# mryndzionek/composable-sdr

Measured on AMD Instinct MI355X. Metric: MS/s CF32 throughput, 256-ch PFB+FM pipeline, higher is better.
Workload: dtype f32; 1 GPU; cfg3: 256-ch firpfbch(m=7,As=80)+dcBlocker+freqdem(kf=0.3) on synthetic CF32, AGC off (-a 0), 262144 frames/step (512 MiB in, 256 MiB out), HBM-resident; channels=256, demod=fm, mix=False, route=fused-256|k_tile256<FM>, preheat_steps=10762, collective=none, rccl_ranks=1

## Files before the change

### composable_sdr_amd/csrc/capi.hip

```cpp
#include "../../include/csdr.h"
#include "csdr_internal.h"
#include "fused.h"

#include <cmath>
#include <cstdio>
#include <cstring>
#include <new>

namespace csdr {
const char *last_error();
}
using namespace csdr;

namespace {

struct DevGuard {
    int prev = -1; bool ok = true;
    DevGuard() = default;
    explicit DevGuard(int dev) { select(dev); }
    void select(int dev) {
        if (hipGetDevice(&prev) != hipSuccess) { ok = false; return; }
        if (dev >= 0 && dev != prev && hipSetDevice(dev) != hipSuccess) ok = false;
    }
    ~DevGuard() { if (prev >= 0) (void)hipSetDevice(prev); }
// ... 983 lines not shown
        h->d_theta = nco_freq_word(pfb_premix_freq(M));
        h->tab_len = nco_period(h->d_theta, 1u << 17);
        if ((r = chain_alloc(h, &h->d_taps, h->taps.size()))) return fail(r);
        CSDR_HIP_CLEAN(hipMemcpy(h->d_taps, h->taps.data(), sizeof(float) * h->taps.size(), hipMemcpyHostToDevice), csdr_chain_destroy(h));
        if (h->tab_len) {
            std::vector<float2> tab(h->tab_len);
            for (uint32_t i = 0; i < h->tab_len; i++) { float c, s; nco_phasor(i * h->d_theta, &c, &s); tab[i] = make_float2(c, s); }
            if ((r = chain_alloc(h, &h->d_nco_tab, h->tab_len))) return fail(r);
            CSDR_HIP_CLEAN(hipMemcpy(h->d_nco_tab, tab.data(), sizeof(float2) * h->tab_len, hipMemcpyHostToDevice), csdr_chain_destroy(h));
        }
        std::vector<float2> tw(M);
        for (uint32_t i = 0; i < M; i++) {
            double a = -2.0 * 3.14159265358979323846 * (double)i / (double)M;
            tw[i] = make_float2((float)std::cos(a), (float)std::sin(a));
        }
        if ((r = chain_alloc(h, &h->d_tw, M))) return fail(r);
        CSDR_HIP_CLEAN(hipMemcpy(h->d_tw, tw.data(), sizeof(float2) * M, hipMemcpyHostToDevice), csdr_chain_destroy(h));
    }
    if (cfg->agc_threshold_db != 0.0f && (r = chain_alloc(h, &h->d_agc, C))) return fail(r);
    if (cfg->demod == CSDR_DEMOD_FM && ((r = chain_alloc(h, &h->d_rp[0], C)) || (r = chain_alloc(h, &h->d_rp[1], C)))) return fail(r);

    const DcParams *dcp = cfg->dc_block ? &h->dc : nullptr;
    const RouteRow *route = route_select(M, h->p, G, cfg->flags, dcp);
    if (route->M == 4096 && (C != M || (cfg->mix && cfg->demod == CSDR_DEMOD_NONE && cfg->agc_threshold_db == 0.0f && !am)))
        route = route_select(M, h->p, G, cfg->flags | CSDR_FLAG_FORCE_GENERIC, dcp);
    if (route->create) {
        const bool agc_on = cfg->agc_threshold_db != 0.0f;
        FusedConfig fc{};
        fc.M = M; fc.p = h->p; fc.C = C; fc.c0 = c0; fc.max_nf = h->max_nf; fc.G = G;
        fc.dc_block = cfg->dc_block != 0; fc.dc = h->dc;
        fc.fm = cfg->demod == CSDR_DEMOD_FM && !agc_on; fc.fm_ref = h->fm_ref;
        fc.mix = cfg->mix != 0 && !agc_on; fc.taps = h->taps.data(); fc.d_theta = h->d_theta; fc.cus = h->n_cus;
        if ((r = route->create(fc, &h->plan))) return fail(r);
        h->path = std::string(route->path_prefix) + h->plan->name() + (G > 1 ? "+interleaved-shard" : "") + (agc_on ? "+agc" : "");
        h->timed_kernel = h->plan->name();
        if (agc_on) {
            const bool tm_possible = !(cfg->flags & CSDR_FLAG_AGC_SEQUENTIAL) && h->max_nf >= 4096u &&
                                     (C % 64u == 0 || (C < 64u && 64u % C == 0));
            h->a_guard = tm_possible ? agc_tail_tm_guard(C) : 0;
            if ((r = chain_alloc(h, &h->d_A, (size_t)C * h->max_nf + 2 * h->a_guard))) return fail(r);
            if (h->a_guard) {
                CSDR_HIP_CLEAN(hipMemset(h->d_A, 0, sizeof(float2) * h->a_guard), csdr_chain_destroy(h));
                CSDR_HIP_CLEAN(hipMemset(h->d_A + h->a_guard + (size_t)C * h->max_nf, 0, sizeof(float2) * h->a_guard), csdr_chain_destroy(h));
            }
            if (cfg->mix && (r = chain_alloc(h, &h->d_B, (size_t)C * h->max_nf))) return fail(r);
        }
    } else {
        h->path = "generic";
        const bool use1024 = G == 1 && pfb1024_supported(M, h->p) && !(cfg->mix && cfg->agc_threshold_db == 0.0f) && !diag_env("CSDR_NO_PFB1024");
        h->timed_kernel = M > 1 ? (use1024 ? "k_pfb1024" : "k_pfb_fir") : "k_dc_apply";
        if (use1024) h->path = "generic+pfb1024";
        if (M > 1) {
            if ((r = chain_alloc(h, &h->d_u, (size_t)(h->p - 1) * M + h->max_nx)) || (r = chain_alloc(h, &h->d_hist_tmp, (size_t)(h->p - 1) * M))) return fail(r);
        }
        if ((r = chain_alloc(h, &h->d_A, h->max_nx)) || (r = chain_alloc(h, &h->d_B, use1024 && h->max_nx < 2048 ? 2048 : h->max_nx))) return fail(r);
        if (M > 1 && cfg->dc_block && (r = dctile_create(h->dc, h->max_nx, &h->dctile))) return fail(r);
        h->mix_identity = M > 1 && G == 1 && C == M && cfg->mix && cfg->demod == CSDR_DEMOD_NONE && cfg->agc_threshold_db == 0.0f &&
                          h->dctile && !(cfg->flags & CSDR_FLAG_NO_MIX_IDENTITY) && !am;
        if (h->mix_identity) {
            if ((r = chain_alloc(h, &h->d_u0, (size_t)(h->p - 1) + h->max_nf)) || (r = chain_alloc(h, &h->d_u0hist, 2 * (h->p - 1)))) return fail(r);
            h->path = "generic+mix-identity"; h->timed_kernel = (M % 4096u == 0) ? "k_dc_fold" : "k_dc_tile";
        }
        h->mix_identity_shard = M > 1 && (G == 2 || G == 4 || G == 8) && (uint64_t)C * G == M && cfg->mix && cfg->demod == CSDR_DEMOD_NONE && cfg->agc_threshold_db == 0.0f &&
                                h->dctile && !(cfg->flags & CSDR_FLAG_NO_MIX_IDENTITY) && !am && M % 4096u == 0 && (M / G) % 512u == 0 &&
                                h->p <= 33u && h->dc.beta > 0.f;
        if (h->mix_identity_shard) {
            if ((r = chain_alloc(h, &h->d_u0hist, 2 * (size_t)(h->p - 1) * G))) return fail(r);
// ... 616 lines not shown
```

### composable_sdr_amd/csrc/fused.h

```cpp
#pragma once
#include "csdr_internal.h"

namespace csdr {

struct FusedConfig {
    uint32_t M, p, C, c0, max_nf;
    uint32_t G = 1;
    bool dc_block; DcParams dc;
    bool fm; float fm_ref;
    bool mix;
    const float *taps;
    uint32_t d_theta;
    uint32_t cus = 256;
};

struct FusedCall {
    const float2 *d_in;
    void *d_out;
    uint32_t nf;
    uint32_t theta0;
    bool indep = false;
    hipEvent_t ev_tail = nullptr;
    bool tile_major = false;
};

struct ChainPlan {
    FusedConfig cfg;
    uint32_t cus;
    uint64_t frames_done = 0;
    int cur = 0;
    void *d_premix = nullptr;
    DeviceBuffers mem;

    explicit ChainPlan(const FusedConfig &c) : cfg(c), cus(c.cus) {}
    virtual ~ChainPlan() = default;

    int process(const FusedCall &call, hipStream_t s, KernelTimer *timer);
    int reset(hipStream_t s) { cur = 0; frames_done = 0; return reset_state(s); }
    void seek(uint64_t frames) { frames_done = frames; }
    virtual const char *name() const = 0;
    virtual bool tile_major_ok(uint32_t nf) const = 0;

    virtual void keep_tail() {}
    virtual bool can_overlap(uint32_t nf) const { (void)nf; return false; }
    virtual bool tail_recorded() const { return false; }
    virtual int status(unsigned *st) { *st = 0; return 0; }
    virtual int trace(unsigned long long *out, uint32_t ntiles) { (void)out; (void)ntiles; return 0; }

protected:
    std::vector<float2> premix_table() const;
    virtual int reset_state(hipStream_t s) = 0;
    virtual int run(const FusedCall &call, void *out, hipStream_t s, KernelTimer *timer) = 0;
};

template <class Plan> int make_plan(const FusedConfig &cfg, ChainPlan **out)
{
    Plan *p = new Plan(cfg);
    if (int r = p->init()) { delete p; return r; }
    *out = p;
    return 0;
}

bool plan256_supported(uint32_t M, uint32_t p);
int  plan256_create(const FusedConfig &cfg, ChainPlan **out);
bool plan64_supported(uint32_t M, uint32_t p);
int  plan64_create(const FusedConfig &cfg, ChainPlan **out);
bool plan1024_supported(uint32_t M, uint32_t p);
int  plan1024_create(const FusedConfig &cfg, ChainPlan **out);
bool plan4096_supported(uint32_t M, uint32_t p);
int  plan4096_create(const FusedConfig &cfg, ChainPlan **out);

int  run256_v2_launch(const void *run_args, bool fm, unsigned G, unsigned nruns, hipStream_t s);
int  run256_v2_blocks_per_cu(bool fm);
// ... 60 lines not shown
```

### composable_sdr_amd/csrc/fused_common.h

```cpp
#pragma once
#include "fused.h"

#include <cmath>
#include <cstdlib>
#include <vector>

namespace csdr {
namespace {

constexpr int M256 = 256;
constexpr int P = 14;
constexpr int NB = 16;
constexpr int FS_X = 272;
constexpr int FS_Z = 289;
constexpr int RS_Z = 18;
constexpr int RS_Y = 17;
constexpr int LDS_F2 = 16 * FS_Z;
constexpr int E_OFF = 4096;
constexpr int LOOKBACK = 10;
constexpr unsigned SPIN_LIMIT = 1u << 24;

typedef unsigned long long u64;
typedef float v2f __attribute__((ext_vector_type(2)));

// ... 320 lines not shown
    return f ? r : make_float2(0.f, 0.f);
}


constexpr int WU = 6;

struct RunSplit {
    uint32_t rps, nslots;
    uint32_t base[8], tiles[8];
};
__host__ __device__ __forceinline__ void run_range(const RunSplit &sp, uint32_t w, uint32_t &first, uint32_t &last)
{
    const uint32_t s = w / sp.rps, i = w - s * sp.rps;
    first = sp.base[s] + (uint32_t)((unsigned long long)i * sp.tiles[s] / sp.rps);
    last = sp.base[s] + (uint32_t)((unsigned long long)(i + 1) * sp.tiles[s] / sp.rps);
}

struct RunArgs {
    TileArgs t;
    RunSplit split;
    PhaseK pk;
    uint32_t nruns;
    float l2beta;
    uint32_t prio_div;
    uint32_t trace_light;
    const float4 *prev_tail;
    uint32_t indep;
    uint32_t pair_align;
    uint32_t wu_batch6;
    uint32_t wu, wu_rot;
    uint32_t tile_step;
    uint32_t nowu;
    float2 *cpre, *side;
};
constexpr int DCFIX_F = 113;

__device__ __forceinline__ float2 wg_sum(float2 v, float2 *red, int tid)
{
#pragma unroll
    for (int d = 32; d >= 1; d >>= 1) { v.x += __shfl_xor(v.x, d); v.y += __shfl_xor(v.y, d); }
    if ((tid & 63) == 0) red[tid >> 6] = v;
    __syncthreads();
    const float2 r = cadd(cadd(red[0], red[1]), cadd(red[2], red[3]));
    __syncthreads();
    return r;
}

__device__ __forceinline__ void row_scan4(float &x0, float &x1, float &x2, float &x3, float &s0, float &s1, float &s2, float &s3,
                                          float b1, float b2, float b4, float b8, float na)
{
    asm volatile(
        "v_mov_b32_e32 %4, %0\n\t"
        "v_mov_b32_e32 %5, %1\n\t"
        "v_mov_b32_e32 %6, %2\n\t"
        "v_mov_b32_e32 %7, %3\n\t"
        "v_fmac_f32_dpp %4, %4, %8 row_shr:1 row_mask:0xf bank_mask:0xf\n\t"
        "v_fmac_f32_dpp %5, %5, %8 row_shr:1 row_mask:0xf bank_mask:0xf\n\t"
        "v_fmac_f32_dpp %6, %6, %8 row_shr:1 row_mask:0xf bank_mask:0xf\n\t"
        "v_fmac_f32_dpp %7, %7, %8 row_shr:1 row_mask:0xf bank_mask:0xf\n\t"
        "v_fmac_f32_dpp %4, %4, %9 row_shr:2 row_mask:0xf bank_mask:0xf\n\t"
        "v_fmac_f32_dpp %5, %5, %9 row_shr:2 row_mask:0xf bank_mask:0xf\n\t"
        "v_fmac_f32_dpp %6, %6, %9 row_shr:2 row_mask:0xf bank_mask:0xf\n\t"
        "v_fmac_f32_dpp %7, %7, %9 row_shr:2 row_mask:0xf bank_mask:0xf\n\t"
        "v_fmac_f32_dpp %4, %4, %10 row_shr:4 row_mask:0xf bank_mask:0xf\n\t"
        "v_fmac_f32_dpp %5, %5, %10 row_shr:4 row_mask:0xf bank_mask:0xf\n\t"
        "v_fmac_f32_dpp %6, %6, %10 row_shr:4 row_mask:0xf bank_mask:0xf\n\t"
// ... 64 lines not shown
```

### composable_sdr_amd/csrc/kernels_fused.hip

```cpp
#include "fused_common.h"
#include <cstring>

namespace csdr {

namespace {

#define STAMP(i) do { if (A.trace && tid == 0) A.trace[(size_t)b * 16 + (i)] = __builtin_amdgcn_s_memtime(); } while (0)

template <bool FM>
__global__ __launch_bounds__(256) void k_tile256(TileArgs A)
{
    __shared__ __attribute__((aligned(16))) float2 R[LDS_F2];
    __shared__ float2 tw_s[M256];
    __shared__ float2 Tt[2][16];
    __shared__ float2 carry_s[2];
    __shared__ unsigned tile_s;

    const int tid = threadIdx.x;
    if (tid == 0) tile_s = atomicAdd(A.ticket, 1u);
    tw_s[tid] = A.tw[tid];
    __syncthreads();
    const unsigned b = tile_s;
    if (b >= A.nb) return;
    STAMP(0);
// ... 256 lines not shown
            if (end < base || sp.tiles[k] < 8 * cus) ok = false;
            base = end;
        }
        if (ok) return sp;
    }
    sp = RunSplit{};
    sp.rps = nruns; sp.nslots = 1; sp.base[0] = 0; sp.tiles[0] = nb;
    return sp;
}

__global__ __launch_bounds__(256) void k_save_tail(const float4 *__restrict__ src, float4 *__restrict__ dst)
{
    const unsigned i = blockIdx.x * 256u + threadIdx.x;
    dst[i] = src[i];
}

__global__ __launch_bounds__(64) void k_shard_gather(const float *__restrict__ src, float *__restrict__ dst, uint32_t c0, uint32_t G, uint32_t rem,
                                                     uint32_t nf, uint32_t t0, uint32_t w)
{
    const uint32_t m = blockIdx.x;
    for (uint32_t i = threadIdx.x; i < rem * w; i += 64) dst[((size_t)m * nf + t0) * w + i] = src[(size_t)(c0 + G * m) * rem * w + i];
}

struct FusedPlan : ChainPlan {
    using ChainPlan::ChainPlan;
    std::string kernel;
    uint32_t max_nb = 0, epoch = 0;
    float *d_taps = nullptr;
    float2 *d_tw = nullptr, *d_wpre = nullptr;
    float2 *d_yhist[2] = {nullptr, nullptr}, *d_vend[2] = {nullptr, nullptr}, *d_rp[2] = {nullptr, nullptr};
    unsigned *d_ticket = nullptr, *d_yflag = nullptr, *d_status = nullptr;
    u64 *d_agg = nullptr, *d_ylast = nullptr;
    float2 *d_cpre = nullptr, *d_side = nullptr, *d_rt = nullptr;
    bool nowu = false;
    u64 *d_trace = nullptr;
    uint32_t run_min_tiles = 1024;
    float slot_weight[8] = {1.f, 1.f, 1.f, 1.f, 1.f, 1.f, 1.f, 1.f};
    uint32_t resident_wgs_v2 = 512;
    bool use_v3 = false;
    float *d_shard_tail = nullptr;
    float4 *d_tail[3] = {nullptr, nullptr, nullptr};
    int tail_w = 0;
    bool tail_valid = false, save_tails = false;
    TileArgs proto;

    int init();
    const char *name() const override { return kernel.c_str(); }
    bool tile_major_ok(uint32_t nf) const override;
    void keep_tail() override { save_tails = cfg.G == 1; }
    bool can_overlap(uint32_t nf) const override;
    bool tail_recorded() const override { return save_tails && tail_valid; }
    int status(unsigned *st) override;
    int trace(unsigned long long *out, uint32_t ntiles) override;
    int reset_state(hipStream_t s) override;
    int run(const FusedCall &call, void *out, hipStream_t s, KernelTimer *timer) override;
    bool v2_call(uint32_t nf) const { return cfg.G == 1 && cfg.c0 == 0 && cfg.C == cfg.M && nf / NB >= run_min_tiles; }
};

int ChainPlan::process(const FusedCall &call, hipStream_t s, KernelTimer *timer)
{
    if (!call.nf) return 0;
    if ((call.tile_major && !tile_major_ok(call.nf)) || (call.indep && !can_overlap(call.nf))) {
        set_error("fused: internal: tile-major output or an independent launch requested from a call that cannot run as one");
        return -1;
    }
    int r = run(call, d_premix ? d_premix : call.d_out, s, timer);
    if (r) return r;
    cur ^= 1;
    frames_done += call.nf;
    if (d_premix) return launch_mix((const float *)d_premix, (float *)call.d_out, cfg.C, cfg.fm ? call.nf : 2 * call.nf, s);
    return 0;
}

std::vector<float2> ChainPlan::premix_table() const
{
    std::vector<float2> wpre(2 * cfg.M);
    for (uint32_t i = 0; i < 2 * cfg.M; i++) {
        float c, s;
        nco_phasor(i * cfg.d_theta, &c, &s);
        wpre[i] = make_float2(c, -s);
// ... 42 lines not shown
int FusedPlan::init()
{
    int r;
    kernel = cfg.fm ? "k_tile256<FM>" : "k_tile256<CF32>";
    max_nb = (cfg.max_nf + NB - 1) / NB;
    if ((r = mem.alloc(&d_taps, sizeof(float) * cfg.M * cfg.p))) return r;
    if ((r = mem.alloc(&d_tw, sizeof(float2) * cfg.M))) return r;
    if ((r = mem.alloc(&d_wpre, sizeof(float2) * 2 * cfg.M))) return r;
    for (int i = 0; i < 2; i++) {
        if ((r = mem.alloc(&d_yhist[i], sizeof(float2) * 13 * cfg.M))) return r;
        if ((r = mem.alloc(&d_vend[i], sizeof(float2)))) return r;
        if ((r = mem.alloc(&d_rp[i], sizeof(float2) * (cfg.G > 1 ? cfg.M : cfg.C)))) return r;
    }
    if (cfg.G > 1 && (r = mem.alloc(&d_shard_tail, sizeof(float2) * cfg.M * NB))) return r;
    for (int i = 0; i < 3; i++) {
        if ((r = mem.alloc(&d_tail[i], sizeof(float4) * 2048 * (WU + 1)))) return r;
        CSDR_HIP(hipMemset(d_tail[i], 0, sizeof(float4) * 2048 * (WU + 1)));
    }
    tail_valid = true;
    if ((r = mem.alloc(&d_ticket, sizeof(unsigned)))) return r;
    if ((r = mem.alloc(&d_status, sizeof(unsigned)))) return r;
    if ((r = mem.alloc(&d_yflag, sizeof(unsigned) * max_nb))) return r;
    if ((r = mem.alloc(&d_agg, sizeof(u64) * 2 * max_nb))) return r;
    if ((r = mem.alloc(&d_ylast, sizeof(u64) * (size_t)cfg.M * max_nb))) return r;
    if (const char *e = diag_env("CSDR_RUN_MIN_TILES")) run_min_tiles = (uint32_t)atol(e);
    if (cfg.mix && (r = mem.alloc(&d_premix, (size_t)cfg.C * cfg.max_nf * (cfg.fm ? 4 : 8)))) return r;
    if (diag_env("CSDR_TRACE")) {
        if ((r = mem.alloc(&d_trace, sizeof(u64) * 16 * max_nb))) return r;
        CSDR_HIP(hipMemset(d_trace, 0, sizeof(u64) * 16 * max_nb));
    }
    nowu = cfg.G == 1 && cfg.c0 == 0 && cfg.C == cfg.M && cfg.dc_block && dc_window_ok(cfg.dc, (DCFIX_F - 1) * 256.0) &&
           !(diag_env("CSDR_NOWU") && atoi(diag_env("CSDR_NOWU")) == 0);
    if (nowu) {
        if ((r = mem.alloc(&d_cpre, sizeof(float2) * 2050))) return r;
        if ((r = mem.alloc(&d_side, sizeof(float2) * 2048 * 4 * DCFIX_F))) return r;
        if ((r = mem.alloc(&d_rt, sizeof(float2) * 2 * DCFIX_F * 4))) return r;
        CSDR_HIP(hipMemset(d_cpre, 0, sizeof(float2) * 2050));
    }
    CSDR_HIP(hipMemcpy(d_taps, cfg.taps, sizeof(float) * cfg.M * cfg.p, hipMemcpyHostToDevice));
    std::vector<float2> tw(cfg.M);
    for (uint32_t k1 = 0; k1 < 16; k1++)
        for (uint32_t b1 = 0; b1 < 16; b1++) {
            const double a = -2.0 * 3.14159265358979323846 * (double)(b1 * k1) / (double)cfg.M;
            tw[16 * k1 + b1] = make_float2((float)std::cos(a), (float)std::sin(a));
        }
    const std::vector<float2> wpre = premix_table();
    CSDR_HIP(hipMemcpy(d_tw, tw.data(), sizeof(float2) * cfg.M, hipMemcpyHostToDevice));
    CSDR_HIP(hipMemcpy(d_wpre, wpre.data(), sizeof(float2) * 2 * cfg.M, hipMemcpyHostToDevice));
    if (nowu) {
        std::vector<float2> rt((size_t)2 * DCFIX_F * 4);
        dc_state_response(cfg, wpre.data(), 15u, (uint32_t)DCFIX_F, 126u, rt.data());
        CSDR_HIP(hipMemcpy(d_rt, rt.data(), sizeof(float2) * rt.size(), hipMemcpyHostToDevice));
    }
    CSDR_HIP(hipMemset(d_status, 0, sizeof(unsigned)));
    CSDR_HIP(hipMemset(d_yflag, 0, sizeof(unsigned) * max_nb));
    CSDR_HIP(hipMemset(d_agg, 0, sizeof(u64) * 2 * max_nb));

    TileArgs &A = proto;
    A = TileArgs{};
    A.taps = d_taps; A.tw = d_tw; A.wpre = d_wpre;
    A.ticket = d_ticket; A.agg = d_agg; A.ylast = d_ylast; A.yflag = d_yflag; A.status = d_status;
    A.c0 = cfg.c0; A.C = cfg.C; A.fm_ref = cfg.fm_ref; A.trace = d_trace;
    const double beta = cfg.dc_block ? (double)cfg.dc.beta : 0.0;
    A.alpha = cfg.dc_block ? (float)(1.0 - beta) : 0.0f;
    A.beta = (float)beta;
    for (int k = 0; k < LOOKBACK + 2; k++) A.wtile[k] = (float)std::pow(beta, 4096.0 * k);
    for (int k = 0; k < 16; k++) A.b16[k] = (float)std::pow(beta, 16.0 * k);
    for (int k = 0; k < 17; k++) A.b256[k] = (float)std::pow(beta, 256.0 * k);
    for (int k = 0; k < 16; k++) A.bj[k] = (float)std::pow(beta, (double)k);
    if (const char *e = diag_env("CSDR_CUS")) { if (atoi(e) > 0 && (uint32_t)atoi(e) < cus) cus = (uint32_t)atoi(e); }
// ... 50 lines not shown
    const uint32_t nb_full = nf / NB;
    const bool shard = c.G > 1;
    if (shard && (uint64_t)c.C * nf * (c.fm ? 4u : 8u) >= (1ull << 32)) { set_error("fused: interleaved shard output of %u frames exceeds 4 GiB", nf); return -1; }
    const bool whole_band = c.G == 1 && c.c0 == 0 && c.C == c.M;
    if ((nb_full >= run_min_tiles && whole_band) || shard) {
        const bool v2 = true;
        const bool v3 = !shard && use_v3;
        kernel = v3 ? (c.fm ? "k_run256v3<FM>" : "k_run256v3<CF32>") : (c.fm ? "k_run256v2<FM>" : "k_run256v2<CF32>");
        if (shard) kernel += "/G" + std::to_string(c.G);
        RunArgs RA{};
        A.nf = nb_full * NB; A.nb = nb_full;
        RA.t = A; RA.pk = phase_consts(c.fm_ref);
        uint32_t nruns = v3 ? cus : resident_wgs_v2;
        if (v3) { if (const char *e = diag_env("CSDR_V3_RUNS")) nruns = (uint32_t)atol(e); }
        if (nruns > A.nb / 8) nruns = A.nb / 8;
        if (nruns < 1) nruns = 1;
        RA.nruns = nruns;
        static const float v2_weight_cf[8] = {1.2f, 0.8f, 1.f, 1.f, 1.f, 1.f, 1.f, 1.f};
        static const float v2_weight_fm[8] = {1.24f, 0.76f, 1.f, 1.f, 1.f, 1.f, 1.f, 1.f};
        const float *v2_weight = c.fm ? v2_weight_fm : v2_weight_cf;
        static const float equal_weight[8] = {1.f, 1.f, 1.f, 1.f, 1.f, 1.f, 1.f, 1.f};
        static const bool pd_equal = diag_env("CSDR_PD_EQUAL") != nullptr;
        RA.split = make_split(A.nb, nruns, cus, (call.indep && pd_equal) ? equal_weight : ((v2 && !diag_env("CSDR_RUN_WEIGHTS")) ? v2_weight : slot_weight));
        { const char *e = diag_env("CSDR_PRIO_ROT"); RA.prio_div = e ? (atoi(e) ? cus : 0u) : (v2 ? 0u : cus); }
        { const char *e = diag_env("CSDR_TRACE"); RA.trace_light = (e && atoi(e) == 2) ? 1u : 0u; }
        { const char *e = diag_env("CSDR_WU"); RA.wu = e ? (uint32_t)atoi(e) : (uint32_t)WU; }
        { const char *e = diag_env("CSDR_WU_ROT"); RA.wu_rot = e ? (uint32_t)atoi(e) : 0u; }
        RA.pair_align = (v2 && (c.fm || diag_env("CSDR_PAIR_ALIGN_CF"))) ? 1u : 0u;
        { const char *e = diag_env("CSDR_WU_BATCH6"); RA.wu_batch6 = e ? (uint32_t)atoi(e) : 1u; }
        RA.l2beta = c.dc_block ? (float)std::log2((double)c.dc.beta) : -1000.0f;
        RA.tile_step = call.tile_major ? c.C * 128u : (uint32_t)NB * (c.fm ? 4u : 8u);
        const bool whole = nf == nb_full * NB;
        RA.indep = call.indep ? 1u : 0u;
        RA.nowu = (nowu && !shard && !v3 && !RA.indep && nruns >= 2 && nruns <= 2048) ? 1u : 0u;
        RA.cpre = d_cpre; RA.side = d_side;
        RA.prev_tail = d_tail[tail_w];
        if (save_tails && !shard && v2 && whole && nb_full >= WU + 1) {
            const int nxt = (tail_w + 1) % 3;
            static const bool nocopy = diag_env("CSDR_PD_NOCOPY") != nullptr;
            if (!nocopy) hipLaunchKernelGGL(k_save_tail, dim3(2048 * (WU + 1) / 256), dim3(256), 0, s,
                                            reinterpret_cast<const float4 *>(call.d_in + (size_t)(nb_full - (WU + 1)) * 4096), d_tail[nxt]);
            if (call.ev_tail) CSDR_HIP(hipEventRecord(call.ev_tail, s));
            tail_w = nxt; tail_valid = true;
        } else tail_valid = false;
        if (timer && (r = timer->begin(s))) return r;
        if (nb_full == 0) {  }
#ifdef CSDR_WITH_RUN256_V3
        else if (v3) { if ((r = run256_v3_launch(&RA, c.fm, nruns, s))) return r; }
#endif
        else if ((r = run256_v2_launch(&RA, c.fm, c.G, nruns, s))) return r;
        if (RA.nowu && nb_full && (r = run256_dcfix_launch(&RA, c.fm, nruns, d_rt, s))) return r;
        if (timer && (r = timer->end(s))) return r;
        const uint32_t rem = nf - nb_full * NB;
        if (rem) {
            if (nb_full) cur ^= 1;
            TileArgs T = proto;
            T.x = call.d_in + (size_t)nb_full * NB * c.M; T.out = A.out;
            if (shard) { T.c0 = 0; T.C = c.M; T.out = d_shard_tail; }
            T.yhist_in = d_yhist[cur]; T.yhist_out = d_yhist[cur ^ 1];
            T.vend_in = d_vend[cur];   T.vend_out = d_vend[cur ^ 1];
            T.rp_in = d_rp[cur];       T.rp_out = d_rp[cur ^ 1];
            if (++epoch == 0) epoch = 1;
            T.epoch = epoch; T.nf = rem; T.nb = 1; T.out_stride = nf; T.out_t0 = nb_full * NB;
            if (shard) { T.out_stride = rem; T.out_t0 = 0; }
            T.parity0 = (uint32_t)((frames_done + nb_full * NB) & 1);
            CSDR_HIP(hipMemsetAsync(d_ticket, 0, sizeof(unsigned), s));
            if (c.fm) hipLaunchKernelGGL(k_tile256<true>, dim3(1), dim3(256), 0, s, T);
            else hipLaunchKernelGGL(k_tile256<false>, dim3(1), dim3(256), 0, s, T);
            if (shard) hipLaunchKernelGGL(k_shard_gather, dim3(c.C), dim3(64), 0, s, (const float *)d_shard_tail, (float *)A.out, c.c0, c.G, rem,
                                          nf, nb_full * NB, c.fm ? 1u : 2u);
        }
    } else {
        kernel = c.fm ? "k_tile256<FM>" : "k_tile256<CF32>";
        tail_valid = false;
        if (++epoch == 0) epoch = 1;
        A.epoch = epoch; A.nf = nf; A.nb = (nf + NB - 1) / NB;
        CSDR_HIP(hipMemsetAsync(d_ticket, 0, sizeof(unsigned), s));
        if (timer && (r = timer->begin(s))) return r;
        if (c.fm) hipLaunchKernelGGL(k_tile256<true>, dim3(A.nb), dim3(256), 0, s, A);
        else hipLaunchKernelGGL(k_tile256<false>, dim3(A.nb), dim3(256), 0, s, A);
        if (timer && (r = timer->end(s))) return r;
    }
    CSDR_HIP(hipGetLastError());
    return 0;
// ... 20 lines not shown
```

### composable_sdr_amd/csrc/kernels_fused_v2.hip

```cpp
#ifndef V2_FM_PACKED
#define V2_FM_PACKED 1
#endif
#ifndef V2_ABLATE
#define V2_ABLATE 0
#endif

#ifndef V2_COLSCAN
#define V2_COLSCAN 0
#endif
#ifndef V2_PAIR
#define V2_PAIR 1
#endif
#ifndef V2_STORE_AUX
#define V2_STORE_AUX ""
#endif
#ifndef V2_PAIR_CF
#define V2_PAIR_CF 0
#endif
#ifndef V2_BAR_E
#define V2_BAR_E 0
#endif
#ifndef V2_PAD
#define V2_PAD 1
#endif
#ifndef V2_SNOP
#define V2_SNOP ""
#endif

#include "fused_v2_common.h"
#include <cstddef>
#include <type_traits>

namespace csdr {
namespace {

constexpr unsigned V2_FSB = 2048u + (V2_PAD ? 128u : 0u);
constexpr int V2_FS2 = (int)V2_FSB / 8;
constexpr int V2_BUF = 16 * V2_FS2;
constexpr int V2_STASH = 2 * V2_BUF;
constexpr int V2_F2 = V2_STASH + 256 + 32 + 256 + (V2_COLSCAN ? 512 : 0);
#define V2_ZSW(f) (V2_PAD ? (((f) >> 1) & 7) : ((f) & 7))
#ifndef V2_RSWN
#define V2_RSWN V2_PAD
#endif
#define V2_RSW(a) (V2_RSWN ? ((a) & 7) : (((a) >> 1) & 7))

struct V2Args {
    RunArgs r;
};

template <bool FM, int G>
__global__ __launch_bounds__(256, 2) void k_run256v2(V2Args VA)
{
    static_assert(G == 1 || G == 2 || G == 4 || G == 8, "interleaved shards: G = 2, 4, 8");
    constexpr int NK1 = 16 / G;
    const RunArgs &RA = VA.r;
    const TileArgs &A = RA.t;
    __shared__ __attribute__((aligned(16))) float2 L[V2_F2];
    float2 *R = L, *ST = L + V2_STASH, *Tt = ST + 256, *red = Tt + 16;
    float2 *tw_s = red + 16;
    float2 *TRc = tw_s + 256, *Ec = TRc + 256;
    (void)TRc; (void)Ec;
    float2 *H = L + V2_BUF;
    float2 *E = ST;
    const int tid = threadIdx.x, j = tid;
    const unsigned w = blockIdx.x;
    unsigned first, last;
    run_range(RA.split, w, first, last);
    if (RA.pair_align) {
        first &= ~1u;
        if (last != A.nb) last &= ~1u;
    }
    const float4 *x4 = reinterpret_cast<const float4 *>(A.x);
    const int col_off = 16 * (j >> 4) + 2 * (((j & 15) >> 1) ^ V2_RSW(j >> 4)) + (j & 1);
    const unsigned goff = V2_RSWN ? dma_offset_rsw(tid) : dma_offset(tid);
    const unsigned wave_u = (unsigned)__builtin_amdgcn_readfirstlane(tid >> 6);
    const unsigned lds_wave = (unsigned)(size_t)(__attribute__((address_space(3))) float2 *)R + V2_FSB * (wave_u >> 1) + 1024u * (wave_u & 1u);

#ifndef V2_TRACE
#define V2_TRACE 0
#endif
#if V2_TRACE
#define V2LSTAMP(i) do { if (A.trace && RA.trace_light && tid == 0) A.trace[(size_t)first * 16 + (i)] = __builtin_amdgcn_s_memrealtime(); } while (0)
#else
#define V2LSTAMP(i) do { } while (0)
#endif
    V2LSTAMP(0);
    const bool cold = w > 0 || RA.indep;
    const int halo = (int)first - 1;
    auto tile_ptr = [&](int t) -> const float4 * { return t >= 0 ? x4 + (size_t)t * 2048 : RA.prev_tail + (size_t)(WU + 1 + t) * 2048; };
    if (first < last) dma_tile<false, 2 * V2_FSB>(x4 + (size_t)first * 2048, goff, lds_wave);
    if (cold) dma_tile<false, 2 * V2_FSB>(tile_ptr(halo), goff, lds_wave + (unsigned)(V2_BUF * 8));
    float h[P];
#pragma unroll
    for (int n = 0; n < P; n++) h[n] = A.taps[(M256 - 1 - j) + n * M256];
    float2 Wa = A.wpre[(A.parity0 & 1) * M256 + j], Wb = A.wpre[((A.parity0 & 1) ^ 1) * M256 + j];
    if (G > 1) {
        const int n = ((j >> 4) * (int)A.c0) & 15;
        const float C1 = 0.92387953251128674f, S1 = 0.38268343236508977f, R2 = 0.70710678118654752f;
// ... 91 lines not shown
    const int st_i = XIDX(tid >> 4), st_j1 = ((tid & 15) - (int)(G > 1 ? A.c0 : 0u)) / G;
    const bool st_own = G == 1 || ((((tid & 15) - (int)A.c0) & (G - 1)) == 0 && (tid & 15) >= (int)A.c0);
    const int st_idx = G == 1 ? (tid & 15) * 16 + st_i : (st_own ? ((st_i / NK1) * NK1 + st_j1) * 16 + st_i : 0);
    if (st_own) ST[st_idx] = (FM && !cold) ? A.rp_in[tid] : make_float2(0.f, 0.f);
    __syncthreads();
    if (FM && cold) {
        w2 = cmul(w2, Wa);
        v2f acc = {0.f, 0.f};
#pragma unroll
        for (int n = P - 1; n >= 0; n--) {
            const float2 s2 = (n == P - 1) ? w2 : wa[NB - 1 - n];
            acc = __builtin_elementwise_fma((v2f){s2.x, s2.y}, (v2f){h[n], h[n]}, acc);
        }
        H[j] = to_f2(acc);
        __syncthreads();
        v2f vv[16];
        if (tid < 16) {
#pragma unroll
            for (int a = 0; a < 16; a++) vv[a] = to_v(H[16 * a + tid]);
            fft16_v(vv);
#pragma unroll
            for (int i = (G > 1 ? 0 : 1); i < 16; i++) vv[i] = cmul_v(vv[i], to_v(tw_s[16 * ((XIDX(i) + (G > 1 ? (int)A.c0 : 0)) & 15) + tid]));
#pragma unroll
            for (int i = 0; i < 16; i++) H[256 + 16 * XIDX(i) + tid] = to_f2(vv[i]);
        }
        __syncthreads();
        if (tid < 16) {
#pragma unroll
            for (int b = 0; b < 16; b++) vv[b] = to_v(H[256 + 16 * (G * (tid % NK1)) + b]);
            fft16_v(vv);
#pragma unroll
            for (int i = 0; i < 16; i++) ST[tid * 16 + i] = to_f2(vv[i]);
            if (G == 1 && RA.nowu) {
                if (tid >= 14) RA.side[((size_t)w * 4 + (tid - 14)) * DCFIX_F] = to_f2(vv[13]);
                else if (tid <= 1) RA.side[((size_t)w * 4 + 2 + tid) * DCFIX_F] = to_f2(vv[2]);
            }
        }
        __syncthreads();
    }

    const v2f Wav = to_v(Wa), Wbv = to_v(Wb);
    const float na = opaque_v(-A.alpha), be = opaque_v(A.beta);
    const float kJ = -A.alpha * exp2f((float)j * RA.l2beta);
    const float b256 = A.b256[1];
    const FmK2 fk = {{opaque_v(9.999993443e-01f), opaque_v(-3.332985938e-01f), opaque_v(1.994656026e-01f), opaque_v(-1.390860826e-01f),
                      opaque_v(9.642146528e-02f), opaque_v(-5.591168255e-02f), opaque_v(2.186254039e-02f), opaque_v(-4.054457881e-03f)},
                     opaque_v(1e-37f), opaque_v(A.fm_ref), opaque_v(RA.pk.hp), opaque_v(RA.pk.pi)};
    const int q = tid, sw = V2_RSW(q & 15);
    const unsigned raw_a = (unsigned)q * 128u + (unsigned)(q >> 4) * (V2_FSB - 2048u) + ((unsigned)sw << 4);
    const int f1 = tid >> 4, b1 = tid & 15;
    const int k1 = tid >> 4, f2 = tid & 15;
    const unsigned x_a = (unsigned)f1 * V2_FSB + (unsigned)b1 * 8u;
    const unsigned zw_a = (unsigned)f1 * V2_FSB + (unsigned)((((b1 >> 1) ^ V2_ZSW(f1)) << 1) | (b1 & 1)) * 8u;
    const unsigned z_a = (unsigned)f2 * V2_FSB + (unsigned)k1 * 128u + ((unsigned)V2_ZSW(f2) << 4);
    const int j1 = k1 % NK1, hb = (G == 8) ? ((k1 >> 1) & 1) : 0;
    const unsigned z_a_g = (unsigned)f2 * V2_FSB + (unsigned)(G * j1) * 128u + ((unsigned)V2_ZSW(f2) << 4);
    const uint32_t voff = ((uint32_t)(G == 1 ? k1 : j1 + 16 * hb) * A.out_stride + A.out_t0 + (uint32_t)f2) * (FM ? 4u : 8u);
    const size_t row16 = (size_t)NK1 * A.out_stride * (FM ? 4u : 8u);
#if V2_TRACE
#define V2STAMP(i) do { if (A.trace && !RA.trace_light && tid == 0) A.trace[(size_t)b_ * 16 + (i)] = __builtin_amdgcn_s_memtime(); } while (0)
#else
#define V2STAMP(i) do { } while (0)
#endif

    float hold[16];
    v2f holdc[V2_PAIR_CF ? 16 : 1];
    auto tile = [&](float2 (&old)[NB], float2 (&nw)[NB], unsigned b_, const int par) {
        unsigned b = (unsigned)__builtin_amdgcn_readfirstlane((int)b_);
        asm volatile("" : "+s"(b));
        char *B = reinterpret_cast<char *>(L) + par * (V2_BUF * 8);
        float2 *Bf = reinterpret_cast<float2 *>(B);
        if (RA.prio_div) {
            if (((b_ - first) + w / RA.prio_div) & 1u) __builtin_amdgcn_s_setprio(1); else __builtin_amdgcn_s_setprio(0);
        }
        V2STAMP(0);
        if (G == 1 && b + 1 == last && tid == 0) {
            if (kernarg_u32_s<offsetof(V2Args, r.nowu)>()) kernarg_ptr_s<offsetof(V2Args, r.cpre)>()[w + 1] = c;
        }
        if (V2_TRACE && A.trace && !RA.trace_light && tid == 0) A.trace[(size_t)b_ * 16 + 15] = __builtin_amdgcn_s_memrealtime();
        bar();
        V2STAMP(1);
#ifdef V2_SELECTIVE_POLICY
        if (!(V2_ABLATE & 1) && b + 1 < last) {
            if (b + 1 + (WU + 1) < last) dma_tile<true, 2 * V2_FSB>(x4 + (size_t)(b + 1) * 2048, goff, lds_wave + (unsigned)(par ^ 1) * (V2_BUF * 8u));
            else dma_tile<false, 2 * V2_FSB>(x4 + (size_t)(b + 1) * 2048, goff, lds_wave + (unsigned)(par ^ 1) * (V2_BUF * 8u));
        }
#else
        if (!(V2_ABLATE & 1) && b + 1 < last) dma_tile<false, 2 * V2_FSB>(x4 + (size_t)(b + 1) * 2048, goff, lds_wave + (unsigned)(par ^ 1) * (V2_BUF * 8u));
#endif
#if V2_COLSCAN
#pragma unroll
        for (int f = 0; f < NB; f++) nw[f] = Bf[V2_FS2 * f + col_off];
        col_run_scan(nw, TRc, A, tid);
        V2STAMP(2);
        bar();
        col_run_carries(TRc, Ec, Tt, A, tid);
        bar();
        V2STAMP(3);
        {
            v2f V = to_v(c);
            const float kj = -A.alpha * A.bj[j & 15];
            const v2f kJv = {kJ, kJ}, bv = {b256, b256}, kjv = {kj, kj};
#pragma unroll
            for (int f = 0; f < NB; f++) {
                v2f y = __builtin_elementwise_fma(V, kJv, to_v(nw[f]));
                nw[f] = to_f2(__builtin_elementwise_fma(to_v(Ec[16 * f + (j >> 4)]), kjv, y));
                V = __builtin_elementwise_fma(V, bv, to_v(Tt[f]));
            }
            c = to_f2(V);
        }
// ... 148 lines not shown
                            if (V2_PAIR && par == 1) asm volatile("s_nop 4\n\tglobal_store_dword %0, %1, %2 offset:-64" V2_STORE_AUX :: "v"(voff), "v"(hold[u]), "s"(rowp) : "memory");
                            asm volatile("s_nop 4\n\tglobal_store_dword %0, %1, %2" V2_STORE_AUX :: "v"(voff), "v"(mq[u]), "s"(rowp) : "memory");
                        }
                    }
                    if (f2 == 15) {
#pragma unroll
                        for (int u = 0; u < NS; u += 2) *reinterpret_cast<v4f *>(stp + u) = (v4f){y[u].x, y[u].y, y[u + 1].x, y[u + 1].y};
                    }
                } else {
#pragma unroll
                    for (int u = 0; u < NS; u++) {
                        const char *rowp = obase + (size_t)XIDX(S0 + u) * row16;
                        asm volatile("s_nop 4\n\tglobal_store_dwordx2 %0, %1, %2\n\ts_nop 1" :: "v"(voff), "v"(y[u]), "s"(rowp) : "memory");
                    }
                }
            };
            if (G == 2) { if (wave_u < 2u) shard_tail(std::integral_constant<int, 0>{}); else shard_tail(std::integral_constant<int, 2>{}); }
            else switch (wave_u) {
                case 0: shard_tail(std::integral_constant<int, 0>{}); break;
                case 1: shard_tail(std::integral_constant<int, 1>{}); break;
                case 2: shard_tail(std::integral_constant<int, 2>{}); break;
                default: shard_tail(std::integral_constant<int, 3>{}); break;
            }
            V2STAMP(14);
            return;
        }
#pragma unroll
        for (int i = 0; i < 8; i++) {
            const v4f v = *reinterpret_cast<const v4f *>(B + (z_a ^ (unsigned)(i << 4)));
            vv[2 * i] = (v2f){v.x, v.y}; vv[2 * i + 1] = (v2f){v.z, v.w};
        }
        if (!(V2_ABLATE & 16)) fft16_v(vv);
        V2STAMP(11);
        if (G == 1 && cold && b - first < 7u && kernarg_u32_s<offsetof(V2Args, r.nowu)>()) {
            float2 *sd = kernarg_ptr_s<offsetof(V2Args, r.side)>() + ((size_t)w * 4) * DCFIX_F + 1 + 16 * (size_t)(b - first) + f2;
            if (k1 >= 14) sd[(k1 - 14) * DCFIX_F] = to_f2(vv[13]);
            else if (k1 <= 1) sd[(2 + k1) * DCFIX_F] = to_f2(vv[2]);
        }
        char *obase = reinterpret_cast<char *>(A.out) + (size_t)b * RA.tile_step;
        if (FM) {
            asm volatile("s_waitcnt vmcnt(0)" ::: "memory");
#pragma unroll
            for (int i = 0; i < 16; i += 4) {
                float2 rp[4], rr[4];
#pragma unroll
                for (int u = 0; u < 4; u += 2) {
                    const v4f sp = *reinterpret_cast<const v4f *>(ST + k1 * 16 + i + u);
                    rp[u] = make_float2(dpp_keep<0x111>(sp.x, vv[i + u].x), dpp_keep<0x111>(sp.y, vv[i + u].y));
                    rp[u + 1] = make_float2(dpp_keep<0x111>(sp.z, vv[i + u + 1].x), dpp_keep<0x111>(sp.w, vv[i + u + 1].y));
                    rr[u] = to_f2(vv[i + u]); rr[u + 1] = to_f2(vv[i + u + 1]);
                }
                float mq_[4];
                float (&mq)[4] = (V2_PAIR && par == 0) ? *reinterpret_cast<float (*)[4]>(&hold[i]) : mq_;
                if (V2_ABLATE & 4) { mq[0] = rp[0].x + rr[0].y; mq[1] = rp[1].y + rr[1].x; mq[2] = rp[2].x + rr[2].y; mq[3] = rp[3].y + rr[3].x; }
                else if (V2_FM_PACKED) fm_quad(rp, rr, fk, mq);
                else {
                    const FmK k1s = {fk.tiny, fk.ref, fk.hp, fk.pi};
#pragma unroll
                    for (int u = 0; u < 4; u++) mq[u] = fm_sample(rp[u], rr[u], k1s);
                }
                if (V2_PAIR && par == 0 && b + 1 < last) continue;
#pragma unroll
                for (int u = 0; u < 4; u++) {
                    const char *rowp = obase + (size_t)XIDX(i + u) * row16;
                    if (V2_ABLATE & 2) asm volatile("" :: "v"(mq[u]), "s"(rowp));
                    else {
                        if (V2_PAIR && par == 1) asm volatile(V2_SNOP "global_store_dword %0, %1, %2 offset:-64" V2_STORE_AUX :: "v"(voff), "v"(hold[i + u]), "s"(rowp) : "memory");
                        asm volatile(V2_SNOP "global_store_dword %0, %1, %2" V2_STORE_AUX :: "v"(voff), "v"(mq[u]), "s"(rowp) : "memory");
                    }
                }
// ... 12 lines not shown
#pragma unroll
                for (int i = 0; i < 16; i++) holdc[i] = vv[i];
            } else {
#pragma unroll
                for (int i = 0; i < 16; i++) {
                    const char *rowp = obase + (size_t)XIDX(i) * row16;
                    if (V2_ABLATE & 2) asm volatile("" :: "v"(vv[i]), "s"(rowp));
                    else {
                        if (V2_PAIR_CF && par == 1) asm volatile(V2_SNOP "global_store_dwordx2 %0, %1, %2 offset:-128" V2_STORE_AUX :: "v"(voff), "v"(holdc[i]), "s"(rowp) : "memory");
                        asm volatile(V2_SNOP "global_store_dwordx2 %0, %1, %2" V2_STORE_AUX :: "v"(voff), "v"(vv[i]), "s"(rowp) : "memory");
                    }
                }
            }
        }
        V2STAMP(14);
    };

    V2LSTAMP(2);
    asm volatile("s_waitcnt vmcnt(0)" ::: "memory");
    V2LSTAMP(3);
    for (unsigned b = first; b < last; b += 2) {
        tile(wa, wb, b, 0);
        if (b + 1 >= last) break;
        tile(wb, wa, b + 1, 1);
    }

    V2LSTAMP(4);
    bar();
    if (FM) {
        const float2 lastY = ST[st_idx];
        if (last == A.nb && st_own) A.rp_out[tid] = lastY;
    }
    if (last == A.nb && tid == 0) A.vend_out[0] = c;
}

}

template <bool FM>
__global__ __launch_bounds__(128) void k_run256_dcfix(V2Args VA, const float2 *__restrict__ Rt)
{
    const RunArgs &RA = VA.r;
    const TileArgs &A = RA.t;
    __shared__ float2 Ys[4][DCFIX_F + 1];
    const unsigned w = blockIdx.x + 1;
    unsigned first, last;
    run_range(RA.split, w, first, last);
    if (RA.pair_align) { first &= ~1u; if (last != A.nb) last &= ~1u; }
    if (first >= last || first <= 1) return;
    const int t = threadIdx.x;
    const float2 c = RA.cpre[w];
    const float2 *R = Rt + (size_t)(A.parity0 & 1u) * DCFIX_F * 4;
    float2 y[4];
    if (t < DCFIX_F) {
#pragma unroll
        for (int ch = 0; ch < 4; ch++) {
            const float2 r = R[t * 4 + ch], s0 = RA.side[((size_t)w * 4 + ch) * DCFIX_F + t];
            y[ch] = make_float2(fmaf(c.x, r.x, fmaf(-c.y, r.y, s0.x)), fmaf(c.x, r.y, fmaf(c.y, r.x, s0.y)));
            Ys[ch][t] = y[ch];
        }
    }
    __syncthreads();
    if (t < 1 || t >= DCFIX_F) return;
    const unsigned b = first + (unsigned)(t - 1) / 16u, f2 = (unsigned)(t - 1) & 15u;
    if (b >= last) return;
    char *obase = reinterpret_cast<char *>(A.out) + (size_t)b * RA.tile_step;
    const FmK fk = {1e-37f, A.fm_ref, RA.pk.hp, RA.pk.pi};
#pragma unroll
    for (int ch = 0; ch < 4; ch++) {
        const size_t off = ((size_t)(126 + ch) * A.out_stride + A.out_t0 + f2) * (FM ? 4u : 8u);
        if (FM) *reinterpret_cast<float *>(obase + off) = fm_sample(Ys[ch][t - 1], y[ch], fk);
        else *reinterpret_cast<float2 *>(obase + off) = y[ch];
    }
}

int run256_dcfix_launch(const void *run_args, bool fm, unsigned nruns, const float2 *Rt, hipStream_t s)
{
    if (nruns < 2) return 0;
    V2Args VA;
    VA.r = *static_cast<const RunArgs *>(run_args);
    if (fm) hipLaunchKernelGGL(k_run256_dcfix<true>, dim3(nruns - 1), dim3(128), 0, s, VA, Rt);
    else hipLaunchKernelGGL(k_run256_dcfix<false>, dim3(nruns - 1), dim3(128), 0, s, VA, Rt);
    return 0;
}

static V2Args make_v2(const void *run_args)
{
    V2Args VA;
    VA.r = *static_cast<const RunArgs *>(run_args);
    return VA;
}

int run256_v2_launch(const void *run_args, bool fm, unsigned G, unsigned nruns, hipStream_t s)
{
    const V2Args VA = make_v2(run_args);
#define V2_LAUNCH(F, GG) hipLaunchKernelGGL((k_run256v2<F, GG>), dim3(nruns), dim3(256), 0, s, VA)
    if (G == 1) { if (fm) V2_LAUNCH(true, 1); else V2_LAUNCH(false, 1); }
    else if (G == 2) { if (fm) V2_LAUNCH(true, 2); else V2_LAUNCH(false, 2); }
    else if (G == 4) { if (fm) V2_LAUNCH(true, 4); else V2_LAUNCH(false, 4); }
    else if (G == 8) { if (fm) V2_LAUNCH(true, 8); else V2_LAUNCH(false, 8); }
    else { set_error("k_run256v2: interleaved shards of stride %u are not built (2, 4, 8)", G); return -1; }
#undef V2_LAUNCH
    return 0;
}

int run256_v2_blocks_per_cu(bool fm)
// ... 9 lines not shown
```

Before: 301,600 MS/s.

## Fuse DC-fix correction into main 256-ch kernel via epoch-tagged cross-block handoff

The separate k_run256_dcfix launch is replaced by default with an in-kernel tail. Each block publishes its carry state as epoch-tagged 64-bit atomics, and the next block spin-waits for it and applies the DC correction from side data held in LDS. This removes a second kernel launch and the global side buffer round trip. In exchange the main kernel uses more LDS and blocks now depend on their predecessors, which risks stalls or deadlock if they are not co-resident. The old separate launch is still available through CSDR_DCFIX_LAUNCH.

```diff
diff --git a/composable_sdr_amd/csrc/capi.hip b/composable_sdr_amd/csrc/capi.hip
--- a/composable_sdr_amd/csrc/capi.hip
+++ b/composable_sdr_amd/csrc/capi.hip
@@ -1039,7 +1039,7 @@
         fc.fm = cfg->demod == CSDR_DEMOD_FM && !agc_on; fc.fm_ref = h->fm_ref;
         fc.mix = cfg->mix != 0 && !agc_on; fc.taps = h->taps.data(); fc.d_theta = h->d_theta; fc.cus = h->n_cus;
         if ((r = route->create(fc, &h->plan))) return fail(r);
-        h->path = std::string(route->path_prefix) + h->plan->name() + (G > 1 ? "+interleaved-shard" : "") + (agc_on ? "+agc" : "");
+        h->path = std::string(route->path_prefix) + h->plan->name() + h->plan->path_suffix() + (G > 1 ? "+interleaved-shard" : "") + (agc_on ? "+agc" : "");
         h->timed_kernel = h->plan->name();
         if (agc_on) {
             const bool tm_possible = !(cfg->flags & CSDR_FLAG_AGC_SEQUENTIAL) && h->max_nf >= 4096u &&
diff --git a/composable_sdr_amd/csrc/fused.h b/composable_sdr_amd/csrc/fused.h
--- a/composable_sdr_amd/csrc/fused.h
+++ b/composable_sdr_amd/csrc/fused.h
@@ -39,6 +39,7 @@
     int reset(hipStream_t s) { cur = 0; frames_done = 0; return reset_state(s); }
     void seek(uint64_t frames) { frames_done = frames; }
     virtual const char *name() const = 0;
+    virtual const char *path_suffix() const { return ""; }
     virtual bool tile_major_ok(uint32_t nf) const = 0;
 
     virtual void keep_tail() {}
diff --git a/composable_sdr_amd/csrc/fused_common.h b/composable_sdr_amd/csrc/fused_common.h
--- a/composable_sdr_amd/csrc/fused_common.h
+++ b/composable_sdr_amd/csrc/fused_common.h
@@ -376,6 +376,7 @@
     uint32_t tile_step;
     uint32_t nowu;
     float2 *cpre, *side;
+    const float2 *rt;
 };
 constexpr int DCFIX_F = 113;
 
diff --git a/composable_sdr_amd/csrc/kernels_fused.hip b/composable_sdr_amd/csrc/kernels_fused.hip
--- a/composable_sdr_amd/csrc/kernels_fused.hip
+++ b/composable_sdr_amd/csrc/kernels_fused.hip
@@ -312,7 +312,8 @@
     unsigned *d_ticket = nullptr, *d_yflag = nullptr, *d_status = nullptr;
     u64 *d_agg = nullptr, *d_ylast = nullptr;
     float2 *d_cpre = nullptr, *d_side = nullptr, *d_rt = nullptr;
-    bool nowu = false;
+    bool nowu = false, dcfix_launch = false;
+    uint32_t run_epoch = 0;
     u64 *d_trace = nullptr;
     uint32_t run_min_tiles = 1024;
     float slot_weight[8] = {1.f, 1.f, 1.f, 1.f, 1.f, 1.f, 1.f, 1.f};
@@ -326,6 +327,7 @@
 
     int init();
     const char *name() const override { return kernel.c_str(); }
+    const char *path_suffix() const override { return nowu && dcfix_launch ? "+dcfix-launch" : ""; }
     bool tile_major_ok(uint32_t nf) const override;
     void keep_tail() override { save_tails = cfg.G == 1; }
     bool can_overlap(uint32_t nf) const override;
@@ -434,10 +436,11 @@
     nowu = cfg.G == 1 && cfg.c0 == 0 && cfg.C == cfg.M && cfg.dc_block && dc_window_ok(cfg.dc, (DCFIX_F - 1) * 256.0) &&
            !(diag_env("CSDR_NOWU") && atoi(diag_env("CSDR_NOWU")) == 0);
     if (nowu) {
-        if ((r = mem.alloc(&d_cpre, sizeof(float2) * 2050))) return r;
-        if ((r = mem.alloc(&d_side, sizeof(float2) * 2048 * 4 * DCFIX_F))) return r;
+        if (const char *e = diag_env("CSDR_DCFIX_LAUNCH")) dcfix_launch = atoi(e) != 0;
+        if ((r = mem.alloc(&d_cpre, sizeof(u64) * 2 * 2050))) return r;
+        if (dcfix_launch && (r = mem.alloc(&d_side, sizeof(float2) * 2048 * 4 * DCFIX_F))) return r;
         if ((r = mem.alloc(&d_rt, sizeof(float2) * 2 * DCFIX_F * 4))) return r;
-        CSDR_HIP(hipMemset(d_cpre, 0, sizeof(float2) * 2050));
+        CSDR_HIP(hipMemset(d_cpre, 0, sizeof(u64) * 2 * 2050));
     }
     CSDR_HIP(hipMemcpy(d_taps, cfg.taps, sizeof(float) * cfg.M * cfg.p, hipMemcpyHostToDevice));
     std::vector<float2> tw(cfg.M);
@@ -554,8 +557,9 @@
         RA.tile_step = call.tile_major ? c.C * 128u : (uint32_t)NB * (c.fm ? 4u : 8u);
         const bool whole = nf == nb_full * NB;
         RA.indep = call.indep ? 1u : 0u;
-        RA.nowu = (nowu && !shard && !v3 && !RA.indep && nruns >= 2 && nruns <= 2048) ? 1u : 0u;
-        RA.cpre = d_cpre; RA.side = d_side;
+        RA.nowu = (nowu && !shard && !v3 && !RA.indep && nruns >= 2 && nruns <= 2048) ? (dcfix_launch ? 2u : 1u) : 0u;
+        RA.cpre = d_cpre; RA.side = d_side; RA.rt = d_rt;
+        if (RA.nowu == 1u) { if (++run_epoch == 0) run_epoch = 1; RA.t.epoch = run_epoch; }
         RA.prev_tail = d_tail[tail_w];
         if (save_tails && !shard && v2 && whole && nb_full >= WU + 1) {
             const int nxt = (tail_w + 1) % 3;
@@ -571,7 +575,7 @@
         else if (v3) { if ((r = run256_v3_launch(&RA, c.fm, nruns, s))) return r; }
 #endif
         else if ((r = run256_v2_launch(&RA, c.fm, c.G, nruns, s))) return r;
-        if (RA.nowu && nb_full && (r = run256_dcfix_launch(&RA, c.fm, nruns, d_rt, s))) return r;
+        if (RA.nowu == 2u && nb_full && (r = run256_dcfix_launch(&RA, c.fm, nruns, d_rt, s))) return r;
         if (timer && (r = timer->end(s))) return r;
         const uint32_t rem = nf - nb_full * NB;
         if (rem) {
diff --git a/composable_sdr_amd/csrc/kernels_fused_v2.hip b/composable_sdr_amd/csrc/kernels_fused_v2.hip
--- a/composable_sdr_amd/csrc/kernels_fused_v2.hip
+++ b/composable_sdr_amd/csrc/kernels_fused_v2.hip
@@ -39,6 +39,7 @@
 constexpr int V2_BUF = 16 * V2_FS2;
 constexpr int V2_STASH = 2 * V2_BUF;
 constexpr int V2_F2 = V2_STASH + 256 + 32 + 256 + (V2_COLSCAN ? 512 : 0);
+constexpr int V2_SIDE = 4 * DCFIX_F;
 #define V2_ZSW(f) (V2_PAD ? (((f) >> 1) & 7) : ((f) & 7))
 #ifndef V2_RSWN
 #define V2_RSWN V2_PAD
@@ -48,6 +49,37 @@
 struct V2Args {
     RunArgs r;
 };
+
+__device__ __forceinline__ void dcfix_table_row(const float2 *Rt, int t, float2 (&r)[4])
+{
+#pragma unroll
+    for (int ch = 0; ch < 4; ch++) r[ch] = t < DCFIX_F ? Rt[t * 4 + ch] : make_float2(0.f, 0.f);
+}
+template <bool FM>
+__device__ __forceinline__ void run256_dcfix_rows(int t, float2 c, const float2 (&r)[4], const float2 *side, float2 *Ys, unsigned first, unsigned last,
+                                                  char *out, uint32_t tile_step, uint32_t out_stride, uint32_t out_t0, const FmK &fk)
+{
+    float2 y[4];
+    if (t < DCFIX_F) {
+#pragma unroll
+        for (int ch = 0; ch < 4; ch++) {
+            const float2 s0 = side[ch * DCFIX_F + t];
+            y[ch] = make_float2(fmaf(c.x, r[ch].x, fmaf(-c.y, r[ch].y, s0.x)), fmaf(c.x, r[ch].y, fmaf(c.y, r[ch].x, s0.y)));
+            Ys[ch * DCFIX_F + t] = y[ch];
+        }
+    }
+    __syncthreads();
+    if (t < 1 || t >= DCFIX_F) return;
+    const unsigned b = first + (unsigned)(t - 1) / 16u, f2 = (unsigned)(t - 1) & 15u;
+    if (b >= last) return;
+    char *obase = out + (size_t)b * tile_step;
+#pragma unroll
+    for (int ch = 0; ch < 4; ch++) {
+        const size_t off = ((size_t)(126 + ch) * out_stride + out_t0 + f2) * (FM ? 4u : 8u);
+        if (FM) *reinterpret_cast<float *>(obase + off) = fm_sample(Ys[ch * DCFIX_F + t - 1], y[ch], fk);
+        else *reinterpret_cast<float2 *>(obase + off) = y[ch];
+    }
+}
 
 template <bool FM, int G>
 __global__ __launch_bounds__(256, 2) void k_run256v2(V2Args VA)
@@ -56,15 +88,20 @@
     constexpr int NK1 = 16 / G;
     const RunArgs &RA = VA.r;
     const TileArgs &A = RA.t;
-    __shared__ __attribute__((aligned(16))) float2 L[V2_F2];
+    __shared__ __attribute__((aligned(16))) float2 L[V2_F2 + (G == 1 ? V2_SIDE : 0)];
     float2 *R = L, *ST = L + V2_STASH, *Tt = ST + 256, *red = Tt + 16;
     float2 *tw_s = red + 16;
     float2 *TRc = tw_s + 256, *Ec = TRc + 256;
     (void)TRc; (void)Ec;
+    float2 *SD = L + V2_F2;
     float2 *H = L + V2_BUF;
     float2 *E = ST;
     const int tid = threadIdx.x, j = tid;
     const unsigned w = blockIdx.x;
+    auto side_put = [&](unsigned nw, int ch, unsigned t, float2 v) {
+        if (nw == 1u) SD[ch * DCFIX_F + (int)t] = v;
+        else kernarg_ptr_s<offsetof(V2Args, r.side)>()[((size_t)w * 4 + (unsigned)ch) * DCFIX_F + t] = v;
+    };
     unsigned first, last;
     run_range(RA.split, w, first, last);
     if (RA.pair_align) {
@@ -222,8 +259,8 @@
 #pragma unroll
             for (int i = 0; i < 16; i++) ST[tid * 16 + i] = to_f2(vv[i]);
             if (G == 1 && RA.nowu) {
-                if (tid >= 14) RA.side[((size_t)w * 4 + (tid - 14)) * DCFIX_F] = to_f2(vv[13]);
-                else if (tid <= 1) RA.side[((size_t)w * 4 + 2 + tid) * DCFIX_F] = to_f2(vv[2]);
+                if (tid >= 14) side_put(RA.nowu, tid - 14, 0u, to_f2(vv[13]));
+                else if (tid <= 1) side_put(RA.nowu, 2 + tid, 0u, to_f2(vv[2]));
             }
         }
         __syncthreads();
@@ -265,7 +302,13 @@
         }
         V2STAMP(0);
         if (G == 1 && b + 1 == last && tid == 0) {
-            if (kernarg_u32_s<offsetof(V2Args, r.nowu)>()) kernarg_ptr_s<offsetof(V2Args, r.cpre)>()[w + 1] = c;
+            const unsigned nw = kernarg_u32_s<offsetof(V2Args, r.nowu)>();
+            if (nw == 1u) {
+                u64 *cp = reinterpret_cast<u64 *>(kernarg_ptr_s<offsetof(V2Args, r.cpre)>()) + 2 * (size_t)(w + 1);
+                const u64 tag = (u64)kernarg_u32_s<offsetof(V2Args, r.t.epoch)>() << 32;
+                __hip_atomic_store(cp, tag | __float_as_uint(c.x), __ATOMIC_RELAXED, __HIP_MEMORY_SCOPE_AGENT);
+                __hip_atomic_store(cp + 1, tag | __float_as_uint(c.y), __ATOMIC_RELAXED, __HIP_MEMORY_SCOPE_AGENT);
+            } else if (nw) kernarg_ptr_s<offsetof(V2Args, r.cpre)>()[w + 1] = c;
         }
         if (V2_TRACE && A.trace && !RA.trace_light && tid == 0) A.trace[(size_t)b_ * 16 + 15] = __builtin_amdgcn_s_memrealtime();
         bar();
@@ -480,10 +523,13 @@
         }
         if (!(V2_ABLATE & 16)) fft16_v(vv);
         V2STAMP(11);
-        if (G == 1 && cold && b - first < 7u && kernarg_u32_s<offsetof(V2Args, r.nowu)>()) {
-            float2 *sd = kernarg_ptr_s<offsetof(V2Args, r.side)>() + ((size_t)w * 4) * DCFIX_F + 1 + 16 * (size_t)(b - first) + f2;
-            if (k1 >= 14) sd[(k1 - 14) * DCFIX_F] = to_f2(vv[13]);
-            else if (k1 <= 1) sd[(2 + k1) * DCFIX_F] = to_f2(vv[2]);
+        if (G == 1 && cold && b - first < 7u) {
+            const unsigned nw = kernarg_u32_s<offsetof(V2Args, r.nowu)>();
+            if (nw) {
+                const unsigned t = 1u + 16u * (b - first) + (unsigned)f2;
+                if (k1 >= 14) side_put(nw, k1 - 14, t, to_f2(vv[13]));
+                else if (k1 <= 1) side_put(nw, 2 + k1, t, to_f2(vv[2]));
+            }
         }
         char *obase = reinterpret_cast<char *>(A.out) + (size_t)b * RA.tile_step;
         if (FM) {
@@ -562,6 +608,45 @@
         if (last == A.nb && st_own) A.rp_out[tid] = lastY;
     }
     if (last == A.nb && tid == 0) A.vend_out[0] = c;
+    V2LSTAMP(5);
+
+    if constexpr (G == 1) {
+        if (cold && first > 1u && first < last && kernarg_u32_s<offsetof(V2Args, r.nowu)>() == 1u) {
+            float2 r[4];
+            dcfix_table_row(kernarg_ptr_s<offsetof(V2Args, r.rt)>() + (size_t)(kernarg_u32_s<offsetof(V2Args, r.t.parity0)>() & 1u) * DCFIX_F * 4, tid, r);
+            const u64 *cp = reinterpret_cast<const u64 *>(kernarg_ptr_s<offsetof(V2Args, r.cpre)>()) + 2 * (size_t)w;
+            u64 g0 = 0, g1 = 0;
+            if (tid == 0) {
+                g0 = __hip_atomic_load(cp, __ATOMIC_RELAXED, __HIP_MEMORY_SCOPE_AGENT);
+                g1 = __hip_atomic_load(cp + 1, __ATOMIC_RELAXED, __HIP_MEMORY_SCOPE_AGENT);
+            }
+            asm volatile("s_waitcnt vmcnt(0)" ::: "memory");
+            if (tid == 0) {
+                const unsigned ep = kernarg_u32_s<offsetof(V2Args, r.t.epoch)>();
+                unsigned spins = 0;
+                bool ok;
+                while (true) {
+                    ok = (unsigned)(g0 >> 32) == ep && (unsigned)(g1 >> 32) == ep;
+                    if (ok) break;
+                    if (++spins > SPIN_LIMIT) { atomicOr(reinterpret_cast<unsigned *>(kernarg_ptr_s<offsetof(V2Args, r.t.status)>()), 4u); break; }
+                    __builtin_amdgcn_s_sleep(2);
+                    g0 = __hip_atomic_load(cp, __ATOMIC_RELAXED, __HIP_MEMORY_SCOPE_AGENT);
+                    g1 = __hip_atomic_load(cp + 1, __ATOMIC_RELAXED, __HIP_MEMORY_SCOPE_AGENT);
+                }
+                red[0] = make_float2(__uint_as_float((unsigned)g0), __uint_as_float((unsigned)g1));
+                red[1] = make_float2(ok ? 1.f : 0.f, 0.f);
+            }
+            __syncthreads();
+            V2LSTAMP(6);
+            if (red[1].x != 0.f) {
+                const FmK k1s = {fk.tiny, fk.ref, fk.hp, fk.pi};
+                run256_dcfix_rows<FM>(tid, red[0], r, SD, SD, first, last, reinterpret_cast<char *>(kernarg_ptr_s<offsetof(V2Args, r.t.out)>()),
+                                      kernarg_u32_s<offsetof(V2Args, r.tile_step)>(), kernarg_u32_s<offsetof(V2Args, r.t.out_stride)>(),
+                                      kernarg_u32_s<offsetof(V2Args, r.t.out_t0)>(), k1s);
+            }
+            V2LSTAMP(7);
+        }
+    }
 }
 
 }
@@ -571,36 +656,17 @@
 {
     const RunArgs &RA = VA.r;
     const TileArgs &A = RA.t;
-    __shared__ float2 Ys[4][DCFIX_F + 1];
+    __shared__ float2 Ys[4][DCFIX_F];
     const unsigned w = blockIdx.x + 1;
     unsigned first, last;
     run_range(RA.split, w, first, last);
     if (RA.pair_align) { first &= ~1u; if (last != A.nb) last &= ~1u; }
     if (first >= last || first <= 1) return;
-    const int t = threadIdx.x;
-    const float2 c = RA.cpre[w];
-    const float2 *R = Rt + (size_t)(A.parity0 & 1u) * DCFIX_F * 4;
-    float2 y[4];
-    if (t < DCFIX_F) {
-#pragma unroll
-        for (int ch = 0; ch < 4; ch++) {
-            const float2 r = R[t * 4 + ch], s0 = RA.side[((size_t)w * 4 + ch) * DCFIX_F + t];
-            y[ch] = make_float2(fmaf(c.x, r.x, fmaf(-c.y, r.y, s0.x)), fmaf(c.x, r.y, fmaf(c.y, r.x, s0.y)));
-            Ys[ch][t] = y[ch];
-        }
-    }
-    __syncthreads();
-    if (t < 1 || t >= DCFIX_F) return;
-    const unsigned b = first + (unsigned)(t - 1) / 16u, f2 = (unsigned)(t - 1) & 15u;
-    if (b >= last) return;
-    char *obase = reinterpret_cast<char *>(A.out) + (size_t)b * RA.tile_step;
     const FmK fk = {1e-37f, A.fm_ref, RA.pk.hp, RA.pk.pi};
-#pragma unroll
-    for (int ch = 0; ch < 4; ch++) {
-        const size_t off = ((size_t)(126 + ch) * A.out_stride + A.out_t0 + f2) * (FM ? 4u : 8u);
-        if (FM) *reinterpret_cast<float *>(obase + off) = fm_sample(Ys[ch][t - 1], y[ch], fk);
-        else *reinterpret_cast<float2 *>(obase + off) = y[ch];
-    }
+    float2 r[4];
+    dcfix_table_row(Rt + (size_t)(A.parity0 & 1u) * DCFIX_F * 4, (int)threadIdx.x, r);
+    run256_dcfix_rows<FM>((int)threadIdx.x, RA.cpre[w], r, RA.side + (size_t)w * 4 * DCFIX_F, &Ys[0][0], first, last,
+                          reinterpret_cast<char *>(A.out), RA.tile_step, A.out_stride, A.out_t0, fk);
 }
 
 int run256_dcfix_launch(const void *run_args, bool fm, unsigned nruns, const float2 *Rt, hipStream_t s)
```

Result: no change. 304,400 MS/s, median of 6 (+0.9%).
